# nuclearbombmods/nbody-cosmological-simulation

Measured on AMD Instinct MI355X. Metric: particle-steps/sec (N=65536 fp64 direct-sum leapfrog), higher is better.
Workload: dtype f64

## Files before the change

### nbody_cosmological_simulation_amd/csrc/nb_force_sym.hip

```cpp
#include "nb_dispatch.h"
#include "nb_force_sym_kernel.h"

namespace {


template <typename T, int D, int KICK>
__global__ void __launch_bounds__(NB_BLOCK)
pack_kernel(T *__restrict__ pos, T *__restrict__ vel, const T *__restrict__ acc, const T *__restrict__ mass,
            T *__restrict__ packed, int n, int np, T half_dt, T dt, T gfac, T pad, int p_begin, int p_end, int spread,
            T far_lim, int far_pe)
{
    const int p = p_begin + blockIdx.x * NB_BLOCK + threadIdx.x;
    if (p >= p_end) return;
    if (p < n) {
#pragma unroll
        for (int k = 0; k < D; ++k) {
            const size_t idx = (size_t)p * D + k;
            T x = pos[idx];
            if (KICK) {
                T v = vel[idx];
                if (KICK == NB_PACK_CLOSE_OPEN) v = axpy_rn<T>(v, acc[idx], half_dt);
                v = axpy_rn<T>(v, acc[idx], half_dt);
                x = axpy_rn<T>(x, v, dt);
                vel[idx] = v;
                pos[idx] = x;
            }
            packed[(size_t)k * np + p] = far_pe ? stage_far_pe<T>(x, far_lim, p) : stage_far<T>(x, far_lim, p);
        }
        packed[(size_t)D * np + p] = gfac * mass[p];
    } else {
#pragma unroll
        for (int k = 0; k < D; ++k) packed[(size_t)k * np + p] = (spread && k == 0) ? pad * (T)(1 + (p - n)) : pad;
        packed[(size_t)D * np + p] = (T)0;
    }
}

#ifndef NB_RED_WAVES_N
#define NB_RED_WAVES_N 16
#endif
constexpr int NB_RED_WAVES = NB_RED_WAVES_N;
template <typename T, int D>
__global__ void __launch_bounds__(64 * NB_RED_WAVES)
reduce_sym_kernel(const double *__restrict__ rowslab, const T *__restrict__ colslab,
                  const int *__restrict__ row_slot0, const int *__restrict__ row_nslots,
                  const int *__restrict__ col_upto, int tile_b, int n, int np,
                  double scale, T *__restrict__ acc, T *__restrict__ vel, T half_dt, int do_kick,
                  T *__restrict__ pos, T *__restrict__ packed, T dt, int blk0, double *__restrict__ sums64,
                  double *__restrict__ mm_part, T *__restrict__ pos_next, T far_lim)
{
    __shared__ double s_part[NB_RED_WAVES][D][64];
    const int lane = threadIdx.x & 63, g = threadIdx.x >> 6;
    const int blk = blk0 + blockIdx.x;
    const int p = blk * 64 + lane;
    const int pc = p < n ? p : n - 1;
    const int J = (blk * 64) / tile_b;
    const int s0 = row_slot0[J], ns = row_nslots[J], total = ns + col_upto[J];
    const int off = blk * 64 + lane - J * tile_b;
    double s[D];
#pragma unroll
    for (int k = 0; k < D; ++k) s[k] = 0.0;
#ifndef NB_RED_UNROLL
#define NB_RED_UNROLL 4
#endif
#pragma unroll NB_RED_UNROLL
    for (int c = g; c < total; c += NB_RED_WAVES) {
        if (c < ns) {
#pragma unroll
            for (int k = 0; k < D; ++k) s[k] += rowslab[((size_t)(s0 + c) * D + k) * tile_b + off];
        } else {
#pragma unroll
            for (int k = 0; k < D; ++k) s[k] += (double)colslab[((size_t)(c - ns) * D + k) * np + pc];
        }
    }
#pragma unroll
    for (int k = 0; k < D; ++k) s_part[g][k][lane] = s[k];
    __syncthreads();
    double mm_lo = __builtin_inf(), mm_hi = -__builtin_inf();
    if (g == 0 && p < n) {
#pragma unroll
        for (int k = 0; k < D; ++k) {
            double t = s_part[0][k][lane];
#pragma unroll
            for (int w = 1; w < NB_RED_WAVES; ++w) t += s_part[w][k][lane];
            const size_t idx = (size_t)p * D + k;
            if (sums64) {
                sums64[idx] = t;
                continue;
            }
            const T a = (T)(t * scale);
            const T a_prev = (do_kick & NB_KICK_OPEN_ON_READ) ? acc[idx] : (T)0;
            acc[idx] = a;
            if (mm_part) {
                const double ad = (double)a;
                mm_lo = (ad != ad || mm_lo != mm_lo) ? __builtin_nan("") : (ad < mm_lo ? ad : mm_lo);
                mm_hi = (ad != ad || mm_hi != mm_hi) ? __builtin_nan("") : (ad > mm_hi ? ad : mm_hi);
            }
            const int kmode = do_kick & NB_KICK_MODE_MASK;
            if (kmode != NB_KICK_NONE) {
                T v = vel[idx];
                if (do_kick & NB_KICK_OPEN_ON_READ) v = axpy_rn<T>(v, a_prev, half_dt);
                v = axpy_rn<T>(v, a, half_dt);
                if (kmode == NB_KICK_CLOSE) {
                    vel[idx] = v;
                } else if (kmode == NB_KICK_CLOSE_OPEN) {
                    v = axpy_rn<T>(v, a, half_dt);
                    const T x = axpy_rn<T>(pos[idx], v, dt);
                    vel[idx] = v;
                    pos[idx] = x;
                    packed[(size_t)k * np + p] = stage_far<T>(x, far_lim, p);
                } else {
                    vel[idx] = v;
                    const T vo = axpy_rn<T>(v, a, half_dt);
                    const T x = axpy_rn<T>(pos[idx], vo, dt);
                    pos_next[idx] = x;
                    packed[(size_t)k * np + p] = stage_far<T>(x, far_lim, p);
                }
            }
        }
    }
    if (mm_part && g == 0) {
#pragma unroll
        for (int off = 32; off >= 1; off >>= 1) {
            const double ol = __shfl_xor(mm_lo, off, 64), oh = __shfl_xor(mm_hi, off, 64);
            mm_lo = (ol != ol || mm_lo != mm_lo) ? __builtin_nan("") : (ol < mm_lo ? ol : mm_lo);
            mm_hi = (oh != oh || mm_hi != mm_hi) ? __builtin_nan("") : (oh > mm_hi ? oh : mm_hi);
        }
        if (lane == 0) { mm_part[2 * blockIdx.x] = mm_lo; mm_part[2 * blockIdx.x + 1] = mm_hi; }
    }
}

__global__ void __launch_bounds__(NB_BLOCK)
finish_sums64_kernel(const double *__restrict__ sums64, double scale, float *__restrict__ acc, long long count)
{
    const long long e = (long long)blockIdx.x * NB_BLOCK + threadIdx.x;
    if (e < count) acc[e] = (float)(sums64[e] * scale);
}

template <typename T, typename TM, int D, int R, bool DIAG, bool UNIFORM>
__device__ __forceinline__ double pe_sweep_f64(const T (&xi)[R][D], const TM (&mi)[R], T (&xj)[R][D], TM (&mj)[R], double eps2,
                                               int mass_dt, int rot_addr, int s_begin, int s_count)
{
    double tsum[R];
#pragma unroll
    for (int r = 0; r < R; ++r) tsum[r] = 0.0;
    double half = 0.5, one = 1.0;
    asm volatile("" : "+v"(half), "+s"(one));
#pragma unroll 1
    for (int s = s_begin; s < s_begin + s_count; ++s) {
#pragma unroll
        for (int rj = 0; rj < R; ++rj) {
#pragma unroll
            for (int ri = 0; ri < R; ++ri) {
                double d[D];
#pragma unroll
                for (int k = 0; k < D; ++k) d[k] = (double)xj[rj][k] - (double)xi[ri][k];
                double q = __builtin_fma(d[D - 1], d[D - 1], eps2);
#pragma unroll
                for (int k = D - 2; k >= 0; --k) q = __builtin_fma(d[k], d[k], q);
                const double y0 = __builtin_amdgcn_rsq(q);
                const double e = __builtin_fma(-(q * y0), y0, one);
                const double c = __builtin_fma(e, half, one);
                if (UNIFORM) {
                    if (DIAG && ri == rj) tsum[rj] = (s == 0) ? tsum[rj] : __builtin_fma(y0, c, tsum[rj]);
                    else tsum[rj] = __builtin_fma(y0, c, tsum[rj]);
                } else {
                    double mp;
                    if constexpr (std::is_same_v<TM, float>) mp = (double)mass_prod_f32(mi[ri], mj[rj], mass_dt);
                    else mp = (double)mi[ri] * (double)mj[rj];
                    const double term = mp * (y0 * c);
                    if (DIAG && ri == rj) tsum[rj] += (s == 0) ? 0.0 : term;
                    else tsum[rj] += term;
                }
            }
#pragma unroll
            for (int k = 0; k < D; ++k) xj[rj][k] = rot1<T>(xj[rj][k], rot_addr);
            if (!UNIFORM) mj[rj] = rot1<TM>(mj[rj], rot_addr);
        }
    }
    double tile = tsum[0];
#pragma unroll
    for (int r = 1; r < R; ++r) tile += tsum[r];
    return DIAG ? 0.5 * tile : tile;
}

template <int D, int R, bool DIAG, bool UNIFORM>
__device__ __forceinline__ double pe_sweep_f32(const float (&xi)[R][D], const float (&mi)[R], f2 (&xj2)[R / 2][D], f2 (&mj2)[R / 2],
                                               float eps2, int mass_dt, int rot_addr, int s_begin, int s_count)
{
    f2 ts2[R / 2];
#pragma unroll
    for (int h = 0; h < R / 2; ++h) ts2[h] = f2{0.0f, 0.0f};
#pragma unroll 1
    for (int s = s_begin; s < s_begin + s_count; ++s) {
#pragma unroll
        for (int h = 0; h < R / 2; ++h) {
#pragma unroll
            for (int ri = 0; ri < R; ++ri) {
                f2 d[D];
#pragma unroll
                for (int k = 0; k < D; ++k) d[k] = xj2[h][k] - xi[ri][k];
                f2 r2 = __builtin_elementwise_fma(d[D - 1], d[D - 1], f2{eps2, eps2});
#pragma unroll
                for (int k = D - 2; k >= 0; --k) r2 = __builtin_elementwise_fma(d[k], d[k], r2);
                f2 y = {__builtin_amdgcn_rsqf(r2.x), __builtin_amdgcn_rsqf(r2.y)};
                if (DIAG && s == 0) {
                    if (2 * h == ri) y.x = 0.0f;
                    if (2 * h + 1 == ri) y.y = 0.0f;
                }
                if (UNIFORM) {
                    ts2[h] = ts2[h] + y;
                } else {
                    f2 mp = mj2[h] * mi[ri];
                    if (mass_dt == NB_F16) mp = f2{round_f16(mp.x), round_f16(mp.y)};
// ... 102 lines not shown
                hipLaunchKernelGGL((pack_kernel<T, D.value, K.value>), dim3(grid), dim3(NB_BLOCK), 0, st, (T *)pos, (T *)vel,
                                   (const T *)acc, (const T *)mass, (T *)packed, n, np, (T)half_dt, (T)dt, (T)gfac, (T)pad, p_begin,
                                   p_end, spread_pad, (T)far_lim, far == NB_FAR_PE ? 1 : 0);
                return hipGetLastError();
            });
        });
    });
}

hipError_t nb_launch_force_sym_f64(const double *packed, const SymWork *work, int nwork, double *rowslab,
                                   double *colslab, int np, int dim, int r, int uniform, int pa_f32, double eps2,
                                   hipStream_t st, NbKernelEvents ev, int rowsplit, int ldsrot)
{
    if (ldsrot && dim == 2 && r == 4 && !pa_f32)
        return nb::pick_bool(rowsplit, [&](auto RS) {
            if (ldsrot == SYM_ROT_DPP)
                return launch_sym_ldsrot<RS.value, SYM_ROT_DPP>(packed, work, nwork, rowslab, colslab, np, uniform, eps2, st, ev);
            return launch_sym_ldsrot<RS.value, SYM_ROT_LDS>(packed, work, nwork, rowslab, colslab, np, uniform, eps2, st, ev);
        });
    if (rowsplit) {
        if (dim != 2 || r != 4) return hipErrorInvalidValue;
        if (pa_f32) return launch_sym_rowsplit<HOOK_F32PAIR>(packed, work, nwork, rowslab, colslab, np, uniform, eps2, (float)eps2, st, ev);
        return launch_sym_rowsplit<HOOK_NONE>(packed, work, nwork, rowslab, colslab, np, uniform, eps2, 1.0f, st, ev);
    }
    return nb::pick<2, 3>(dim, [&](auto D) {
        if (pa_f32)
            return nb::pick<2, 4>(r, [&](auto R) {
                return launch_sym_u<double, D.value, R.value, HOOK_F32PAIR>(packed, work, nwork, rowslab, colslab, np, uniform, eps2,
                                                                            nullptr, (float)eps2, st, ev);
            });
        return nb::pick<1, 2, 4>(r, [&](auto R) {
            return launch_sym_u<double, D.value, R.value, HOOK_NONE>(packed, work, nwork, rowslab, colslab, np, uniform, eps2, nullptr,
                                                                     1.0f, st, ev);
        });
    });
}

hipError_t nb_launch_force_sym_f32(const float *packed, const SymWork *work, int nwork, double *rowslab,
                                   float *colslab, int np, int dim, int r, int uniform, int hook, float eps2,
                                   const GridTables *tab, float G, float mass_value, int levels, hipStream_t st,
                                   NbKernelEvents ev)
{
    return nb::pick<2, 3>(dim, [&](auto D) {
        return nb::pick<2, 4>(r, [&](auto R) {
            return nb::pick<HOOK_NONE, HOOK_BF16, HOOK_F16, HOOK_GRID>(hook, [&](auto H) {
                return launch_sym_u<float, D.value, R.value, H.value>(packed, work, nwork, rowslab, colslab, np, uniform, eps2, tab, G,
                                                                      st, ev, mass_value, levels);
            });
        });
    });
}

hipError_t nb_launch_potential_sym(const void *packed, const SymWork *work, int nwork, double *part, int np, int dim,
                                   int r, int is_f64, int f32_terms, int mass_dt, double eps2, int uniform, hipStream_t st)
{
    const float e32 = (float)eps2;
    return nb::pick<2, 3>(dim, [&](auto D) {
        return nb::pick<2, 4>(r, [&](auto R) {
            auto launch = [&](auto real, auto F32T) {
                using T = typename decltype(real)::type;
                return nb::pick_bool(uniform, [&](auto U) {
                    hipLaunchKernelGGL((potential_sym_kernel<T, D.value, R.value, F32T.value, U.value>), dim3(nwork), dim3(NB_BLOCK),
                                       0, st, (const T *)packed, work, part, np, eps2, e32, mass_dt);
                    return hipGetLastError();
                });
            };
            if (is_f64) return nb::pick_bool(f32_terms, [&](auto F32T) { return launch(nb::real_tag<double>{}, F32T); });
            return launch(nb::real_tag<float>{}, std::true_type{});
        });
    });
}

hipError_t nb_launch_finish_sums64(const double *sums64, double scale, float *acc, int64_t count, hipStream_t st)
{
    hipLaunchKernelGGL(finish_sums64_kernel, dim3((unsigned)((count + NB_BLOCK - 1) / NB_BLOCK)), dim3(NB_BLOCK), 0, st, sums64,
                       scale, acc, (long long)count);
    return hipGetLastError();
}

hipError_t nb_launch_reduce_sym(const double *rowslab, const void *colslab, const int *row_slot0,
                                const int *row_nslots, const int *col_upto, int tile_b, int n,
                                int np, int dim, int is_f64, double scale, void *acc, void *vel, double half_dt,
                                int do_kick, void *pos, void *packed, double dt, hipStream_t st, int p_begin, int p_end,
                                double *sums64, double *mm_part, void *pos_next, int far)
{
    const double far_lim = nb_far_limit(far, is_f64);
    if ((do_kick & NB_KICK_MODE_MASK) == NB_KICK_CLOSE_SPEC && !pos_next) return hipErrorInvalidValue;
    if (p_end < 0 || p_end > n) p_end = n;
    if (p_end <= p_begin) return hipSuccess;
    const int blk0 = p_begin / 64;
    const int grid = (p_end + 63) / 64 - blk0;
    return nb::pick<2, 3>(dim, [&](auto D) {
        return nb::pick_real(is_f64, [&](auto real) {
            using T = typename decltype(real)::type;
            hipLaunchKernelGGL((reduce_sym_kernel<T, D.value>), dim3(grid), dim3(64 * NB_RED_WAVES), 0, st, rowslab,
                               (const T *)colslab, row_slot0, row_nslots, col_upto, tile_b, n, np, scale, (T *)acc, (T *)vel,
                               (T)half_dt, do_kick, (T *)pos, (T *)packed, (T)dt, blk0, sums64, mm_part, (T *)pos_next, (T)far_lim);
            return hipGetLastError();
        });
    });
}

#ifdef NB_WG_TRACE
extern "C" int nb_debug_wg_trace(unsigned long long *host, int nwg)
{
    if (nwg > NB_WG_TRACE_MAX) nwg = NB_WG_TRACE_MAX;
    if (hipDeviceSynchronize() != hipSuccess) return -1;
    return hipMemcpyFromSymbol(host, HIP_SYMBOL(nb_wg_trace_buf), sizeof(unsigned long long) * 8 * (size_t)nwg) == hipSuccess ? nwg : -1;
}
#endif
```

### nbody_cosmological_simulation_amd/csrc/nb_internal.h

```cpp
#pragma once
#include <hip/hip_runtime.h>
#include <stdint.h>

#include "../../include/nbody_amd.h"

constexpr int NB_BLOCK = 256;
constexpr int NB_TJ = 256;
constexpr int NB_MAX_LUT = 4096;
constexpr int NB_LUT_MIN = 256;
#ifndef NB_REC_LEVELS
#define NB_REC_LEVELS 32
#endif

enum { HOOK_NONE = 0, HOOK_BF16 = 1, HOOK_F16 = 2, HOOK_GRID = 3,
       HOOK_F32PAIR = 4 ,
       HOOK_AT_RUN_TIME = 5  };

struct GridTables {
    float thr[NB_MAX_LUT + 1];
    float lut[NB_MAX_LUT];
    float qval[NB_MAX_LUT];
    float lmin, lmax, range;
    float r2max;
    float est_a, est_b;
// ... 15 lines not shown
{
    int p = NB_LUT_MIN;
    while (p < levels) p <<= 1;
    return p;
}
inline size_t nb_lut_lds_bytes(int levels) { return 2 * (size_t)(nb_lut_pad(levels) + 1) * sizeof(float); }

struct PruneState {
    unsigned int box_min[3];
    unsigned int box_max[3];
    unsigned long long far;
    unsigned long long lb[2];
    int count;
    int nan_flag;
    int seeded;
    float c[3];
    float rho_m;
    float rho_prev;
    int pair_i, pair_j;
    unsigned int rho_cur;
    unsigned int scan_done;
    unsigned long long best_i, best_j;
};

struct ForceGeom {
    int n;
    int j_begin;
    int j_end;
    int chunk_len;
    int nchunks;
    int r;
};

struct SymWork {
    int tile_i;
    int jt_begin, jt_end;
    int slot;
    int slot_stride;
    int col_ord;
    int s_begin;
    int s_count;
};

enum NbKick {
    NB_KICK_NONE = 0,
    NB_KICK_CLOSE = 1,
    NB_KICK_CLOSE_OPEN = 2,
    NB_KICK_CLOSE_SPEC = 3
};
constexpr int NB_KICK_MODE_MASK = 3;
constexpr int NB_KICK_OPEN_ON_READ = 4;
enum NbPackKick { NB_PACK_NONE = 0, NB_PACK_OPEN = 1, NB_PACK_CLOSE_OPEN = 2 };

struct NbKernelEvents {
    hipEvent_t start = nullptr, stop = nullptr;
};

enum NbFar { NB_FAR_OFF = 0, NB_FAR_FORCE = 1, NB_FAR_PE = 2 };
constexpr double NB_FAR_F64 = 1.2e153;
constexpr float NB_FAR_F32 = 1.2e18f;
inline double nb_far_limit(int far, bool f64_pairs)
{
    if (far == NB_FAR_OFF) return __builtin_inf();
    if (far == NB_FAR_PE && !f64_pairs) return __builtin_inf();
    return f64_pairs ? NB_FAR_F64 : (double)NB_FAR_F32;
}

hipError_t nb_launch_pack(void *pos, void *vel, const void *acc, const void *mass, void *packed, int n, int np,
                          int dim, int is_f64, int kick , double half_dt, double dt, double gfac, int f32_pairs,
                          hipStream_t st, int p_begin = 0, int p_end = -1 ,
                          int spread_pad = 0 ,
                          int far = NB_FAR_FORCE );
hipError_t nb_launch_force_sym_f64(const double *packed, const SymWork *work, int nwork, double *rowslab,
                                   double *colslab, int np, int dim, int r, int uniform, int pa_f32, double eps2,
                                   hipStream_t st, NbKernelEvents ev = {}, int rowsplit = 0 ,
                                   int ldsrot = 0 );
hipError_t nb_launch_force_sym_f32(const float *packed, const SymWork *work, int nwork, double *rowslab,
                                   float *colslab, int np, int dim, int r, int uniform, int hook, float eps2,
                                   const GridTables *tab, float G, float mass_value, int levels, hipStream_t st,
                                   NbKernelEvents ev = {});
hipError_t nb_launch_potential_sym(const void *packed, const SymWork *work, int nwork, double *part, int np, int dim,
                                   int r, int is_f64, int f32_terms, int mass_dt , double eps2,
                                   int uniform , hipStream_t st);
hipError_t nb_launch_final_sum(const double *part, int count, double *out, hipStream_t st);
hipError_t nb_launch_reduce_sym(const double *rowslab, const void *colslab, const int *row_slot0,
                                const int *row_nslots, const int *col_upto, int tile_b, int n,
                                int np, int dim, int is_f64, double scale, void *acc, void *vel, double half_dt,
                                int do_kick ,
                                void *pos, void *packed, double dt, hipStream_t st,
                                int p_begin = 0, int p_end = -1 ,
                                double *sums64 = nullptr ,
                                double *mm_part = nullptr ,
                                void *pos_next = nullptr , int far = NB_FAR_FORCE );
hipError_t nb_launch_finish_sums64(const double *sums64, double scale, float *acc, int64_t count, hipStream_t st);

hipError_t nb_launch_force_f64(const double *pos, const double *mass, double *partial, const ForceGeom &g,
                               int dim, int pair_dt, int qhook, double G, double eps2_py, float eps2_pair,
                               hipStream_t st);
hipError_t nb_launch_force_f32(const float *pos, const float *mass, double *partial, const ForceGeom &g,
                               int dim, int hook, int pa, float G, float eps2, const GridTables *tab, int levels,
                               hipStream_t st, unsigned long long *bin_out = nullptr );
hipError_t nb_launch_force_sym_f32_bins(const float *packed, const SymWork *work, int nwork, double *rowslab,
                                        float *colslab, int np, int dim, int r, int uniform, float eps2,
                                        const GridTables *tab, float G, float mass_value, int levels,
                                        unsigned long long *bin_out, int bin_n, hipStream_t st);
hipError_t nb_launch_grid_quantize_safe_tab(const float *in, float *out, int64_t count, int levels, float min_val,
                                            const double *bounds, GridTables *tab, hipStream_t st);
hipError_t nb_launch_r2max_tables(const float *pos, const ForceGeom &g, int dim, float eps2, GridTables *tab, int levels,
                                  float G, float min_val, int allow_fast, hipStream_t st);
hipError_t nb_launch_r2max(const float *pos, const ForceGeom &g, int dim, float eps2, GridTables *tab,
                           hipStream_t st);
hipError_t nb_launch_r2max_pruned(const float *pos, int n, int dim, float eps2, float *cand, float *rho,
                                  PruneState *ps, GridTables *tab, hipStream_t st);
hipError_t nb_launch_r2max_tracked(const float *pos, int n, int dim, float eps2, float *cand, int *cand_idx, PruneState *ps,
                                   GridTables *tab, int levels, float G, float min_val, int allow_fast, hipStream_t st);
hipError_t nb_launch_grid_tables(GridTables *tab, int levels, float G, float eps2, float min_val,
                                 PruneState *ps , hipStream_t st, int allow_fast = 1);
hipError_t nb_launch_d2bins(const float *pos, int n, int dim, float eps2, const GridTables *tab,
                            int16_t *bins, hipStream_t st, int i0 = 0, int i1 = -1 );

hipError_t nb_launch_reduce(const double *partial, int nchunks, int64_t count, void *acc, int is_f64,
                            void *vel, double half_dt, int do_kick ,
                            void *pos, double dt, hipStream_t st);
hipError_t nb_launch_axpy(void *y, const void *x, double scalar, int64_t count, int is_f64, hipStream_t st);
hipError_t nb_launch_kick_drift(void *pos, void *vel, const void *acc, double half_dt, double dt,
                                int64_t count, int is_f64, hipStream_t st);
hipError_t nb_launch_kick_a32(void *pos, void *vel, const void *acc, double half_dt, double dt, int64_t count,
                              int vel_f64, int pos_f64, int drift, hipStream_t st);
hipError_t nb_launch_convert(const void *in, int in_dt, void *out, int out_dt, int64_t count, hipStream_t st);

hipError_t nb_launch_force_quant_step(float *acc, int64_t count, int levels, double *mn_mx, double *partials,
                                      int16_t *bins, float *vel, float *pos, double half_dt, double dt,
                                      int kick ,
                                      float *packed ,
                                      int np, int dim, hipStream_t st);
hipError_t nb_launch_force_quant_bins(const float *in, float *out, int64_t count, int levels, const double *mn_mx,
                                      int16_t *bins, hipStream_t st);

hipError_t nb_launch_kinetic(const void *vel, const void *mass, int n, int dim, int is_f64, int vel_f32_logical,
                             int half_pa, int mass_dt , double *scratch, double *out,
                             hipStream_t st);
hipError_t nb_launch_potential(const void *pos, const void *mass, const ForceGeom &g, int dim, int is_f64,
                               int pa_f32, int mass_dt , int half_pa, double eps2_py, float eps2_half,
                               double *scratch, double *out, hipStream_t st);

hipError_t nb_launch_cast_hook(const void *in, int in_dt, void *out, int mode, int64_t count, hipStream_t st);
constexpr int NB_MINMAX_BLOCKS = 2048;
hipError_t nb_launch_minmax_generic(const void *in, int is_f64, int64_t count, int log_clamped, double min_val,
                                    double *mn_mx , double *partials, hipStream_t st);
hipError_t nb_launch_grid_quantize(const void *in, void *out, int is_f64, int64_t count, int levels,
                                   const double *mn_mx, hipStream_t st);
hipError_t nb_launch_grid_quantize_safe(const void *in, void *out, int is_f64, int64_t count, int levels,
                                        double min_val, const double *mn_mx, hipStream_t st);

struct NbMetricsArgs {
    const void *pos, *vel, *mass;
    int n, dim;
    int storage_f64;
    int arith_f64;
    int num_bins;
    const float *edges;
    double max_radius;
    int kth;
    double G;
    int radius_only;
    void *scratch;
    double *out;
};
size_t nb_metrics_scratch_bytes(int n, int num_bins);
size_t nb_sort_temp_bytes(int n, int key64);
hipError_t nb_sort_keys(void *tmp, size_t tmp_bytes, const void *kin, void *kout, int n, int key64, hipStream_t st);
hipError_t nb_sort_pairs(void *tmp, size_t tmp_bytes, const void *kin, void *kout, const int *vin, int *vout, int n,
                         int key64, hipStream_t st);
hipError_t nb_launch_metrics(const NbMetricsArgs &a, hipStream_t st);

size_t nb_p2p_handle_bytes();
// ... 102 lines not shown
```

### nbody_cosmological_simulation_amd/csrc/nb_plan.cpp

```cpp
#include "nb_plan.h"

#include <algorithm>
#include <cmath>
#include <cstdlib>

namespace {
int env_int(const char *name, int dflt)
{
    const char *e = getenv(name);
    return e ? atoi(e) : dflt;
}
}

NbKnobs nb_read_knobs()
{
    NbKnobs k;
    k.sym = env_int("NB_SYM", -1);
    k.sym_r = env_int("NB_SYM_R", 0);
    k.sym_cl = std::max(0, env_int("NB_SYM_CL", 0));
    k.sym_split = env_int("NB_SYM_SPLIT", 0);
    if (k.sym_split < 1 || k.sym_split > 16) k.sym_split = 0;
    k.sym_rowsplit = env_int("NB_SYM_ROWSPLIT", -1);
    if (k.sym_rowsplit > 8) k.sym_rowsplit = -1;
    k.tail_pieces = env_int("NB_SYM_TAIL", 0);
    if (k.tail_pieces != 2 && k.tail_pieces != 4 && k.tail_pieces != 8 && k.tail_pieces != 16) k.tail_pieces = 0;
    k.sym_rot = env_int("NB_SYM_ROT", -1);
    if (k.sym_rot < 0 || k.sym_rot > 2) k.sym_rot = -1;
    k.r_onesided = env_int("NB_R", 0);
    k.no_prune = getenv("NB_NO_PRUNE") != nullptr;
    k.no_track = env_int("NB_NO_TRACK", 0) != 0;
    k.no_pe_sym = getenv("NB_NO_PE_SYM") != nullptr;
    k.no_uniform = getenv("NB_NO_UNIFORM") != nullptr;
    k.no_smalln = getenv("NB_NO_SMALLN") != nullptr;
    k.no_grid_fast = getenv("NB_NO_GRID_FAST") != nullptr;
    k.no_p2p = getenv("NB_NO_P2P") != nullptr;
    k.no_p2p_kick = getenv("NB_P2P_NO_KICK") != nullptr;
    k.no_small_fuse = getenv("NB_NO_SMALL_FUSE") != nullptr;
    k.no_spec = getenv("NB_NO_SPEC") != nullptr;
    k.no_x64 = getenv("NB_NO_X64") != nullptr;
    k.no_red_mm = getenv("NB_NO_RED_MM") != nullptr;
    k.small_max = std::max(0, env_int("NB_SMALL_MAX", 0));
    k.small_lanes = env_int("NB_SMALL_LANES", 0);
    if (k.small_lanes != 16 && k.small_lanes != 32 && k.small_lanes != 64) k.small_lanes = 0;
    return k;
}

void nb_plan_sym(const PlanInput &in, const NbKnobs &knobs, SymPlanHost &sp)
{
    sp = SymPlanHost();
    const int n = in.n, dim = in.dim, P = in.nranks;
    const bool is_f64 = in.is_f64;
    const bool tiny = is_f64 && dim == 2 && n <= 2816;
    const int sym_from = dim == 3 ? (is_f64 ? 8192 : 4096) : (is_f64 ? 5120 : 1024);
    int want = (tiny || n >= sym_from) ? 1 : 0;
    if (knobs.sym >= 0) want = knobs.sym;
    if (!want || ((in.flags & NB_FLAG_NO_COMM) && want < 2)) return;
    if (is_f64 && in.mode != NB_FLOAT64) return;
    sp.r = tiny ? 1 : (n >= 20480 || is_f64) ? 4 : 2;
    if ((knobs.sym_r == 1 && is_f64 && dim == 2) || knobs.sym_r == 2 || knobs.sym_r == 4) sp.r = knobs.sym_r;
    sp.tile_b = 64 * sp.r;
    const int T = (n + sp.tile_b - 1) / sp.tile_b;
    const int SR = (T + 3) / 4;
    sp.tiles = SR * 4;
    sp.np = sp.tiles * sp.tile_b;
    const size_t el = is_f64 ? sizeof(double) : sizeof(float);
    if (SR < P) return;
    {
        const long long rows_max = (SR + P - 1) / P;
        const long long entries_max = knobs.sym_split ? rows_max * knobs.sym_split
                                                      : rows_max + 7 * std::min<long long>(rows_max, 2LL * in.cus);
        if ((size_t)dim * sp.np * el * (size_t)entries_max > (size_t)48 << 30) return;
    }

    std::vector<int> ord(SR, -1);
    sp.row_slot0.assign(sp.tiles, 0);
    sp.row_nslots.assign(sp.tiles, 0);
    long long owned_pairs = 0;
    int nrows = 0;
    for (int S = 0; S < SR; ++S) {
        const int k = S % (2 * P);
        const int owner = k < P ? k : 2 * P - 1 - k;
        if (owner == in.rank) {
            ord[S] = nrows++;
            for (int w = 0; w < 4; ++w) owned_pairs += std::max(0, T - (4 * S + w));
        }
    }
    const long long target_items = is_f64 ? 2048 : 4096;
    int cl = (int)(owned_pairs / target_items / 4);
    cl = std::max(1, std::min(cl, 16));
    if (knobs.sym_cl > 0) cl = knobs.sym_cl;
    sp.cl = cl;

    const long long wg_slots = 4LL * in.cus;
    std::vector<int> nch_of(SR, 0), split_of(SR, 1);
    long long items = 0;
    for (int S = 0; S < SR; ++S)
        if (ord[S] >= 0) { nch_of[S] = (T - 4 * S + cl - 1) / cl; items += nch_of[S]; }
    int rowsplit = 0;
    if (knobs.sym_split) {
        for (int S = 0; S < SR; ++S) split_of[S] = knobs.sym_split;
    } else if (sp.r == 4 && items < 1000) {
        int pieces = 4;
        {
            const double t_step[4] = {0.70, 0.60, 0.62, 0.55};
            double best = 1e30;
            for (int nsp : {2, 3, 4, 5, 6, 8}) {
                if (items >= 500 && nsp != 4) continue;
                const long long wgs = items * nsp, rounds = (wgs + in.cus - 1) / in.cus;
                const double cost = rounds * ((64 + nsp - 1) / nsp + 1) * t_step[std::min<long long>(rounds, 4) - 1] +
                                    0.3 * 5.0 * (double)wgs / in.cus;
                if (cost < best) { best = cost; pieces = nsp; }
            }
            if (is_f64 && dim == 2 && cl == 1 && knobs.sym_rowsplit != 0) {
                long long rows_units = 0;
                for (int S = 0; S < SR; ++S)
                    if (ord[S] >= 0) for (int w = 0; w < 4; ++w) rows_units += std::max(0, T - (4 * S + w));
                for (int nsp : {1, 2, 3, 4}) {
                    const long long wgs = rows_units * nsp, rounds = (wgs + in.cus - 1) / in.cus;
                    const double cost = rounds * ((64 + 4 * nsp - 1) / (4 * nsp) + 1) * t_step[std::min<long long>(rounds, 4) - 1] +
                                        0.5 * 2.0 * (double)wgs / in.cus;
                    if (cost < best) { best = cost; rowsplit = nsp; }
                }
            }
// ... 77 lines not shown
```

### nbody_cosmological_simulation_amd/csrc/nb_plan.h

```cpp
#pragma once
#include <vector>

#include "nb_internal.h"

#ifndef NB_SYM_ROT_DEFAULT
#define NB_SYM_ROT_DEFAULT 2
#endif

struct NbKnobs {
    int sym = -1;
    int sym_r = 0;
    int sym_cl = 0;
    int sym_split = 0;
    int sym_rowsplit = -1;
    int tail_pieces = 0;
    int sym_rot = -1;
    int r_onesided = 0;
    bool no_prune = false;
    bool no_track = false;
    bool no_pe_sym = false;
    bool no_uniform = false;
    bool no_smalln = false;
    int small_max = 0;
    int small_lanes = 0;
    bool no_grid_fast = false;
    bool no_p2p = false;
    bool no_red_mm = false;
    bool no_x64 = false;
    bool no_small_fuse = false;
    bool no_p2p_kick = false;
    bool no_spec = false;
};
NbKnobs nb_read_knobs();

struct SymPlanHost {
    bool enabled = false;
    int r = 2, tile_b = 128, tiles = 0, np = 0, nslots = 0, ncol = 0, cl = 1;
    int rowsplit = 0;
    std::vector<SymWork> work;
    std::vector<int> row_slot0, row_nslots, col_upto;
    size_t col_bytes = 0, row_bytes = 0, packed_bytes = 0;
};

struct PlanInput {
    int n = 0, dim = 2, mode = 0, flags = 0, rank = 0, nranks = 1;
    bool is_f64 = true;
    bool multi = false;
    int cus = 256;
};

void nb_plan_sym(const PlanInput &in, const NbKnobs &knobs, SymPlanHost &out);
```

### nbody_cosmological_simulation_amd/csrc/nb_step.cpp

```cpp
#include <algorithm>
#include <cstring>

#include "nb_state.h"

namespace nbhost {

struct NbTuning {
    int onesided_r1_max_n = 8192;
    int onesided_target_wgs = 1024;
    int prune_min_n = 8192;
    int track_min_n = 3072;
    int red_mm_max_blocks = 1024;
    int small_max_f64 = 4096;
    int small_max_f32 = 3072;
    int small_fuse_tables_max_n = 2048;
};
static const NbTuning g_tune{};

int small_max_n(bool is_f64) { return is_f64 ? g_tune.small_max_f64 : g_tune.small_max_f32; }

int onesided_r(int n, const NbKnobs &knobs)
{
    if (knobs.r_onesided == 1 || knobs.r_onesided == 2 || knobs.r_onesided == 4)
        return knobs.r_onesided;
// ... 250 lines not shown
            if (int rc = comm_allreduce_max_u32(s, &s->tab->r2max_bits)) return rc;
    }
    HIPCHK(nb_launch_grid_tables(s->tab, L, G, e.eps2, min_val, prune ? s->prune_state : nullptr, s->stream, allow_fast(s)));
    s->prune_seeded = prune;
    return NB_OK;
}

int launch_pairs(nb_sim *s, const EvalRequest &rq, const Eval &e)
{
    const nb_config &c = s->cfg;
    const auto &sp = s->sym;
    const bool grid = e.hook == HOOK_GRID;
    const int L = grid ? mode_levels(c) : 0;
    unsigned long long *bin_out = (rq.bins && grid) ? s->bin_out : nullptr;
    int slot;
    if (!e.used_sym) {
        if (int rc = prof_begin(s, &slot)) return rc;
        if (s->is_f64)
            HIPCHK(nb_launch_force_f64((const double *)s->pos, (const double *)s->mass, s->partial, s->geom, c.dim, e.pair_dt,
                                       e.hook, c.G, c.softening_sq, e.eps2, s->stream));
        else
            HIPCHK(nb_launch_force_f32((const float *)s->pos, (const float *)s->mass, s->partial, s->geom, c.dim, e.hook,
                                       e.pair_dt, (float)c.G, e.eps2, s->tab, L, s->stream, bin_out));
        s->last_kernel = s->is_f64 ? "force_f64_kernel" : "force_f32_kernel";
        return prof_end(s, slot);
    }
    const int pa_f32 = s->is_f64 && e.pair_dt == NB_F32;
    if (!rq.packed_ready) {
        const double gfac = s->is_f64 ? c.G : (grid ? 1.0 : (double)(float)c.G);
        HIPCHK(nb_launch_pack(s->pos, s->vel, s->acc, s->mass, sp.packed, c.n, sp.np, c.dim, s->is_f64, NB_PACK_NONE, 0.0, 0.0,
                              gfac, pa_f32, s->stream, 0, -1, 0, grid ? NB_FAR_OFF : NB_FAR_FORCE));
    }
    if (int rc = prof_begin(s, &slot, false)) return rc;
    if (s->is_f64) {
        HIPCHK(nb_launch_force_sym_f64((const double *)sp.packed, sp.work, sp.nwork, sp.rowslab, (double *)sp.colslab, sp.np,
                                       c.dim, sp.r, s->mass_uniform, pa_f32, c.softening_sq, s->stream, prof_events(s, slot),
                                       sp.rowsplit ? 1 : 0, s->knobs.sym_rot >= 0 ? s->knobs.sym_rot : NB_SYM_ROT_DEFAULT));
        s->last_kernel = "force_sym_kernel<double";
        return NB_OK;
    }
    const bool uniform = grid ? (s->mass_uniform && sp.r != 2) : e.sym_uniform;
    if (bin_out)
        HIPCHK(nb_launch_force_sym_f32_bins((const float *)sp.packed, sp.work, sp.nwork, sp.rowslab, (float *)sp.colslab, sp.np,
                                            c.dim, sp.r, uniform, e.eps2, s->tab, (float)c.G, (float)s->mass_value, L, bin_out,
                                            c.n, s->stream));
    else
        HIPCHK(nb_launch_force_sym_f32((const float *)sp.packed, sp.work, sp.nwork, sp.rowslab, (float *)sp.colslab, sp.np,
                                       c.dim, sp.r, uniform, e.hook, e.eps2, s->tab, (float)c.G, (float)s->mass_value, L,
                                       s->stream, prof_events(s, slot)));
    s->last_kernel = "force_sym_kernel<float";
    return NB_OK;
}

int reduce_and_exchange(nb_sim *s, const EvalRequest &rq, Eval &e, EvalResult *res)
{
    const nb_config &c = s->cfg;
    const int64_t cnt = nd(s);
    const bool p2p = e.multi && (e.x64 ? p2p_use_x64(s, cnt) : p2p_use(s, cnt));
    void *red_out = p2p ? nb_p2p_data() : (rq.bins ? s->staging : s->acc);
    if (e.x64 && !p2p && !s->sums64) HIPCHK(hipMalloc((void **)&s->sums64, (size_t)cnt * sizeof(double)));
    double *sums64 = e.x64 ? (p2p ? (double *)nb_p2p_data() : s->sums64) : nullptr;
    if (p2p)
        if (int rc = p2p_claim_buffer(s)) return rc;
    const bool fuse_kick = rq.kick && !e.multi && !e.fq;
    int kmode = kick_mode(fuse_kick, rq.open_next);
    if (rq.open_on_read && !(fuse_kick && e.used_sym))
        return fail(NB_ERR_INVALID, "internal: a step started from speculative positions needs the kick-fusing pair-symmetric reduction");
    if (!e.used_sym) {
        HIPCHK(nb_launch_reduce(s->partial, s->geom.nchunks, cnt, red_out, s->is_f64, s->vel, c.dt / 2, kmode, s->pos, c.dt,
                                s->stream));
        site_set(res, "reduce", kmode);
    } else {
        const auto &sp = s->sym;
        if (e.sym_uniform) e.scale = s->is_f64 ? c.G * s->mass_value : (double)((float)c.G * (float)s->mass_value);
        const bool spec = kmode == NB_KICK_CLOSE && rq.spec_next && !grid_mode(c.mode);
        if (spec) {
            if (!s->pos_alt) HIPCHK(hipMalloc(&s->pos_alt, (size_t)cnt * (s->is_f64 ? 8 : 4)));
            kmode = NB_KICK_CLOSE_SPEC;
        }
        if (rq.open_on_read) kmode |= NB_KICK_OPEN_ON_READ;
        HIPCHK(nb_launch_reduce_sym(sp.rowslab, sp.colslab, sp.row_slot0, sp.row_nslots, sp.col_upto, sp.tile_b, c.n, sp.np,
                                    c.dim, s->is_f64, e.scale, red_out, s->vel, c.dt / 2, kmode, s->pos, sp.packed, c.dt,
                                    s->stream, 0, -1, sums64, e.red_mm ? s->scalars + 8 : nullptr, s->pos_alt,
                                    grid_mode(c.mode) ? NB_FAR_OFF : NB_FAR_FORCE));
        site_set(res, "reduce_sym", kmode);
        if (spec) { s->spec_open = true; s->spec_kind = 2; s->spec_dt = c.dt; }
    }
    e.kicked = fuse_kick;
    res->opened = (kmode & NB_KICK_MODE_MASK) == NB_KICK_CLOSE_OPEN;
    if (p2p) {
        NbP2PKick kk{};
        kk.scale = e.scale;
        if (e.x64) kk.f64_to_f32 = 1;
        else if (rq.kick && !e.fq && !s->knobs.no_p2p_kick) {
            kk.mode = kick_mode(true, rq.open_next);
            kk.dim = c.dim; kk.np = e.used_sym ? s->sym.np : 0;
            kk.vel = s->vel; kk.pos = s->pos; kk.packed = e.used_sym ? (void *)s->sym.packed : nullptr;
            kk.half_dt = c.dt / 2; kk.dt = c.dt;
            kk.far_lim = nb_far_limit(grid_mode(c.mode) ? NB_FAR_OFF : NB_FAR_FORCE, s->is_f64);
            e.kicked = true;
            res->opened = rq.open_next;
        }
        HIPCHK(nb_p2p_allreduce(s->acc, (size_t)cnt, s->is_f64 || e.x64, p2p_step_timeout_s(), s->stream, &kk));
        if (kk.mode != NB_KICK_NONE) site_set(res, "p2p", kk.mode);
        s->used_p2p = true;
    } else if (e.x64) {
        if (int rc = comm_allreduce_sum(s, s->sums64, (size_t)cnt, true)) return rc;
        HIPCHK(nb_launch_finish_sums64(s->sums64, e.scale, (float *)s->acc, cnt, s->stream));
    } else if (e.multi) {
        if (int rc = comm_allreduce_sum(s, s->acc, (size_t)cnt, s->is_f64)) return rc;
    }
    return NB_OK;
}

int force_quant_finish(nb_sim *s, const EvalRequest &rq, Eval &e, EvalResult *res)
{
    const nb_config &c = s->cfg;
    const int km = kick_mode(rq.kick, rq.open_next);
    if (e.red_mm)
        HIPCHK(nb_launch_force_quant_finish((float *)s->acc, nd(s), mode_levels(c), s->scalars + 8, (c.n + 63) / 64, s->scalars,
                                            s->fbins, (float *)s->vel, (float *)s->pos, c.dt / 2, c.dt, km, s->stream,
                                            (float *)s->sym.packed, s->sym.np, c.dim));
    else
        HIPCHK(nb_launch_force_quant_step((float *)s->acc, nd(s), mode_levels(c), s->scalars, s->scalars + 8, s->fbins,
                                          (float *)s->vel, (float *)s->pos, c.dt / 2, c.dt, km,
                                          e.used_sym ? (float *)s->sym.packed : nullptr, s->sym.np, c.dim, s->stream));
    const bool packed = km == NB_KICK_CLOSE_OPEN && e.used_sym;
    site_set(res, "fq_finish", km, packed ? (e.red_mm ? ",packed,red_mm" : ",packed") : (e.red_mm ? ",red_mm" : ""));
    e.kicked = rq.kick;
    res->opened = rq.open_next;
    return NB_OK;
}

}

int force_eval(nb_sim *s, EvalRequest rq, EvalResult *result)
{
    if (!s->have_pos || !s->have_mass) return fail(NB_ERR_INVALID, "positions and masses must be set first");
    rq.open_next = rq.kick && rq.open_next;
    EvalResult unread;
    EvalResult *res = result ? result : &unread;
    *res = EvalResult{};
    Eval e = resolve_eval(s);
    if (e.multi && !s->comm) return fail(NB_ERR_COMM, "nranks > 1 but nb_comm_init was not called");
    if (e.multi)
        if (int rc = comm_check(s)) return rc;
    if (e.shard && rq.kick) return fail(NB_ERR_INVALID, "NB_FLAG_NO_COMM handles cannot step");
    if (e.generic) return force_eval_generic(s, rq, e, res);
    s->last_generic = false;
    if (rq.bins) e.fq = e.red_mm = false;
    if (e.hook == HOOK_GRID)
        if (int rc = grid_prepare(s, e, false)) return rc;
    if (int rc = launch_pairs(s, rq, e)) return rc;
    if (int rc = reduce_and_exchange(s, rq, e, res)) return rc;
    if (e.fq)
        if (int rc = force_quant_finish(s, rq, e, res)) return rc;
    if (rq.kick && !e.kicked) {
        if (rq.may_defer) res->deferred = true;
        else {
            HIPCHK(nb_launch_axpy(s->vel, s->acc, s->cfg.dt / 2, nd(s), s->is_f64, s->stream));
            snprintf(res->site, sizeof res->site, "axpy");
        }
    }
    if (rq.bins) return NB_OK;
    s->logical[3] = acc_logical_dtype(s);
    s->have_acc = true;
    return NB_OK;
// ... 271 lines not shown
```

Baseline: 57.65 million.

## Add multi-chain reduce_sym kernel with per-wave independent accumulators and unrolled loads

Adds a new reduce_sym_chains kernel in which each wave keeps CH independent partial-sum chains and issues U batches of slab loads before adding. This exposes more memory-level parallelism and shortens dependent add chains in the row/column slab reduction. It is selected by default (4 waves, 4 chains, 2 unrolls for fp64), with the classic kernel still available through an env knob. Fewer waves per block and more registers per thread may reduce occupancy. The reduction is a small part of the step next to the O(N^2) force pass.

```diff
diff --git a/nbody_cosmological_simulation_amd/csrc/nb_force_sym.hip b/nbody_cosmological_simulation_amd/csrc/nb_force_sym.hip
--- a/nbody_cosmological_simulation_amd/csrc/nb_force_sym.hip
+++ b/nbody_cosmological_simulation_amd/csrc/nb_force_sym.hip
@@ -39,6 +39,7 @@
 #define NB_RED_WAVES_N 16
 #endif
 constexpr int NB_RED_WAVES = NB_RED_WAVES_N;
+constexpr int NB_RED_SHAPE_F64 = 402, NB_RED_SHAPE_F32 = 401;
 template <typename T, int D>
 __global__ void __launch_bounds__(64 * NB_RED_WAVES)
 reduce_sym_kernel(const double *__restrict__ rowslab, const T *__restrict__ colslab,
@@ -129,6 +130,225 @@
     }
 }
 
+template <typename T, int D>
+struct RedSlot {
+    double r[D];
+    T c[D];
+};
+template <int D>
+struct RedSlot<double, D> {
+    double r[D];
+};
+
+template <int KIND, typename T, int D>
+__device__ __forceinline__ void red_load(RedSlot<T, D> &v, int c, const double *__restrict__ rowslab,
+                                         const T *__restrict__ colslab, int s0, int ns, int tile_b, int np, int off, int pc)
+{
+    const bool row = KIND == 1 || (KIND == 0 && c < ns);
+    if (row) {
+#pragma unroll
+        for (int k = 0; k < D; ++k) v.r[k] = rowslab[((size_t)(s0 + c) * D + k) * tile_b + off];
+    } else if constexpr (std::is_same_v<T, double>) {
+#pragma unroll
+        for (int k = 0; k < D; ++k) v.r[k] = colslab[((size_t)(c - ns) * D + k) * np + pc];
+    } else {
+#pragma unroll
+        for (int k = 0; k < D; ++k) v.c[k] = colslab[((size_t)(c - ns) * D + k) * np + pc];
+    }
+}
+
+template <int KIND, typename T, int D>
+__device__ __forceinline__ void red_add(double (&s)[D], const RedSlot<T, D> &v, int c, int ns)
+{
+    if constexpr (std::is_same_v<T, double>) {
+#pragma unroll
+        for (int k = 0; k < D; ++k) s[k] += v.r[k];
+    } else {
+        const bool row = KIND == 1 || (KIND == 0 && c < ns);
+        if (row) {
+#pragma unroll
+            for (int k = 0; k < D; ++k) s[k] += v.r[k];
+        } else {
+#pragma unroll
+            for (int k = 0; k < D; ++k) s[k] += (double)v.c[k];
+        }
+    }
+}
+
+template <int KIND, typename T, int D, int CH, int U>
+__device__ __forceinline__ void red_trip(double (&s)[CH][D], int base, const double *__restrict__ rowslab,
+                                         const T *__restrict__ colslab, int s0, int ns, int tile_b, int np, int off, int pc)
+{
+    RedSlot<T, D> v[U][CH];
+#pragma unroll
+    for (int u = 0; u < U; ++u)
+#pragma unroll
+        for (int j = 0; j < CH; ++j) red_load<KIND, T, D>(v[u][j], base + 16 * u + j, rowslab, colslab, s0, ns, tile_b, np, off, pc);
+#pragma unroll
+    for (int u = 0; u < U; ++u)
+#pragma unroll
+        for (int j = 0; j < CH; ++j) red_add<KIND, T, D>(s[j], v[u][j], base + 16 * u + j, ns);
+}
+
+template <typename T>
+__device__ __forceinline__ T red_finish(double t, double scale, int do_kick, size_t idx, int k, int p, int np, T v0, T x0,
+                                        T a_prev, T half_dt, T dt, T far_lim, T *__restrict__ acc, T *__restrict__ vel,
+                                        T *__restrict__ pos, T *__restrict__ packed, T *__restrict__ pos_next)
+{
+    const T a = (T)(t * scale);
+    acc[idx] = a;
+    const int kmode = do_kick & NB_KICK_MODE_MASK;
+    if (kmode != NB_KICK_NONE) {
+        T v = v0;
+        if (do_kick & NB_KICK_OPEN_ON_READ) v = axpy_rn<T>(v, a_prev, half_dt);
+        v = axpy_rn<T>(v, a, half_dt);
+        if (kmode == NB_KICK_CLOSE) {
+            vel[idx] = v;
+        } else if (kmode == NB_KICK_CLOSE_OPEN) {
+            v = axpy_rn<T>(v, a, half_dt);
+            const T x = axpy_rn<T>(x0, v, dt);
+            vel[idx] = v;
+            pos[idx] = x;
+            packed[(size_t)k * np + p] = stage_far<T>(x, far_lim, p);
+        } else {
+            vel[idx] = v;
+            const T vo = axpy_rn<T>(v, a, half_dt);
+            const T x = axpy_rn<T>(x0, vo, dt);
+            pos_next[idx] = x;
+            packed[(size_t)k * np + p] = stage_far<T>(x, far_lim, p);
+        }
+    }
+    return a;
+}
+
+__device__ __forceinline__ void red_mm_take(double &mm_lo, double &mm_hi, double ad)
+{
+    mm_lo = (ad != ad || mm_lo != mm_lo) ? __builtin_nan("") : (ad < mm_lo ? ad : mm_lo);
+    mm_hi = (ad != ad || mm_hi != mm_hi) ? __builtin_nan("") : (ad > mm_hi ? ad : mm_hi);
+}
+
+template <typename T, int D, int CH, int U>
+__global__ void __launch_bounds__(64 * (16 / CH))
+reduce_sym_chains_kernel(const double *__restrict__ rowslab, const T *__restrict__ colslab,
+                         const int *__restrict__ row_slot0, const int *__restrict__ row_nslots,
+                         const int *__restrict__ col_upto, int tile_b, int n, int np,
+                         double scale, T *__restrict__ acc, T *__restrict__ vel, T half_dt, int do_kick,
+                         T *__restrict__ pos, T *__restrict__ packed, T dt, int blk0, double *__restrict__ sums64,
+                         double *__restrict__ mm_part, T *__restrict__ pos_next, T far_lim)
+{
+    constexpr int NW = 16 / CH;
+    constexpr int FD = NW == 1 ? D : 1;
+    static_assert(NW == 1 || NW >= D, "wave k finishes component k");
+    __shared__ double s_part[NW == 1 ? 1 : 16][D][64];
+    __shared__ double s_acc[NW == 1 ? 1 : D][64];
+    const int lane = threadIdx.x & 63, w = threadIdx.x >> 6, g0 = w * CH;
+    const int blk = blk0 + blockIdx.x;
+    const int p = blk * 64 + lane;
+    const int pc = p < n ? p : n - 1;
+    const int J = (blk * 64) / tile_b;
+    const int s0 = row_slot0[J], ns = row_nslots[J], total = ns + col_upto[J];
+    const int off = blk * 64 + lane - J * tile_b;
+
+    const bool fin = p < n && (NW == 1 || w < D);
+    const int kmode = do_kick & NB_KICK_MODE_MASK;
+    T v0[FD], x0[FD], a_prev[FD];
+#pragma unroll
+    for (int f = 0; f < FD; ++f) {
+        const size_t idx = (size_t)pc * D + (NW == 1 ? f : (w < D ? w : 0));
+        v0[f] = (fin && !sums64 && kmode != NB_KICK_NONE) ? vel[idx] : (T)0;
+        x0[f] = (fin && !sums64 && (kmode == NB_KICK_CLOSE_OPEN || kmode == NB_KICK_CLOSE_SPEC)) ? pos[idx] : (T)0;
+        a_prev[f] = (fin && !sums64 && (do_kick & NB_KICK_OPEN_ON_READ)) ? acc[idx] : (T)0;
+    }
+
+    double s[CH][D];
+#pragma unroll
+    for (int j = 0; j < CH; ++j)
+#pragma unroll
+        for (int k = 0; k < D; ++k) s[j][k] = 0.0;
+    for (int base = g0; base < total; base += 16 * U) {
+        const int last = base + 16 * (U - 1) + CH - 1;
+        if (last < ns) {
+            red_trip<1, T, D, CH, U>(s, base, rowslab, colslab, s0, ns, tile_b, np, off, pc);
+        } else if (base >= ns && last < total) {
+            red_trip<2, T, D, CH, U>(s, base, rowslab, colslab, s0, ns, tile_b, np, off, pc);
+        } else {
+            RedSlot<T, D> v[U][CH];
+#pragma unroll
+            for (int u = 0; u < U; ++u)
+#pragma unroll
+                for (int j = 0; j < CH; ++j) {
+                    const int c = base + 16 * u + j;
+                    if (c < total) red_load<0, T, D>(v[u][j], c, rowslab, colslab, s0, ns, tile_b, np, off, pc);
+                }
+#pragma unroll
+            for (int u = 0; u < U; ++u)
+#pragma unroll
+                for (int j = 0; j < CH; ++j) {
+                    const int c = base + 16 * u + j;
+                    if (c < total) red_add<0, T, D>(s[j], v[u][j], c, ns);
+                }
+        }
+    }
+
+    double t[FD];
+    if constexpr (NW == 1) {
+#pragma unroll
+        for (int k = 0; k < D; ++k) {
+            t[k] = s[0][k];
+#pragma unroll
+            for (int j = 1; j < 16; ++j) t[k] += s[j][k];
+        }
+    } else {
+#pragma unroll
+        for (int j = 0; j < CH; ++j)
+#pragma unroll
+            for (int k = 0; k < D; ++k) s_part[g0 + j][k][lane] = s[j][k];
+        __syncthreads();
+        if (w < D) {
+            t[0] = s_part[0][w][lane];
+#pragma unroll
+            for (int g = 1; g < 16; ++g) t[0] += s_part[g][w][lane];
+        }
+    }
+
+    double mm_lo = __builtin_inf(), mm_hi = -__builtin_inf();
+    if (fin) {
+#pragma unroll
+        for (int f = 0; f < FD; ++f) {
+            const int k = NW == 1 ? f : w;
+            const size_t idx = (size_t)p * D + k;
+            if (sums64) {
+                sums64[idx] = t[f];
+                continue;
+            }
+            const T a = red_finish<T>(t[f], scale, do_kick, idx, k, p, np, v0[f], x0[f], a_prev[f], half_dt, dt, far_lim, acc,
+                                      vel, pos, packed, pos_next);
+            if (mm_part) {
+                if (NW == 1 || w == 0) red_mm_take(mm_lo, mm_hi, (double)a);
+                else s_acc[w][lane] = (double)a;
+            }
+        }
+    }
+    if (mm_part) {
+        if constexpr (NW > 1) {
+            __syncthreads();
+            if (w == 0 && p < n && !sums64) {
+#pragma unroll
+                for (int k = 1; k < D; ++k) red_mm_take(mm_lo, mm_hi, s_acc[k][lane]);
+            }
+        }
+        if (w == 0) {
+#pragma unroll
+            for (int o = 32; o >= 1; o >>= 1) {
+                const double ol = __shfl_xor(mm_lo, o, 64), oh = __shfl_xor(mm_hi, o, 64);
+                mm_lo = (ol != ol || mm_lo != mm_lo) ? __builtin_nan("") : (ol < mm_lo ? ol : mm_lo);
+                mm_hi = (oh != oh || mm_hi != mm_hi) ? __builtin_nan("") : (oh > mm_hi ? oh : mm_hi);
+            }
+            if (lane == 0) { mm_part[2 * blockIdx.x] = mm_lo; mm_part[2 * blockIdx.x + 1] = mm_hi; }
+        }
+    }
+}
+
 __global__ void __launch_bounds__(NB_BLOCK)
 finish_sums64_kernel(const double *__restrict__ sums64, double scale, float *__restrict__ acc, long long count)
 {
@@ -397,7 +617,7 @@
                                 const int *row_nslots, const int *col_upto, int tile_b, int n,
                                 int np, int dim, int is_f64, double scale, void *acc, void *vel, double half_dt,
                                 int do_kick, void *pos, void *packed, double dt, hipStream_t st, int p_begin, int p_end,
-                                double *sums64, double *mm_part, void *pos_next, int far)
+                                double *sums64, double *mm_part, void *pos_next, int far, int shape)
 {
     const double far_lim = nb_far_limit(far, is_f64);
     if ((do_kick & NB_KICK_MODE_MASK) == NB_KICK_CLOSE_SPEC && !pos_next) return hipErrorInvalidValue;
@@ -405,13 +625,25 @@
     if (p_end <= p_begin) return hipSuccess;
     const int blk0 = p_begin / 64;
     const int grid = (p_end + 63) / 64 - blk0;
+    if (shape == NB_RED_AUTO) shape = is_f64 ? NB_RED_SHAPE_F64 : NB_RED_SHAPE_F32;
     return nb::pick<2, 3>(dim, [&](auto D) {
         return nb::pick_real(is_f64, [&](auto real) {
             using T = typename decltype(real)::type;
-            hipLaunchKernelGGL((reduce_sym_kernel<T, D.value>), dim3(grid), dim3(64 * NB_RED_WAVES), 0, st, rowslab,
-                               (const T *)colslab, row_slot0, row_nslots, col_upto, tile_b, n, np, scale, (T *)acc, (T *)vel,
-                               (T)half_dt, do_kick, (T *)pos, (T *)packed, (T)dt, blk0, sums64, mm_part, (T *)pos_next, (T)far_lim);
-            return hipGetLastError();
+            if (shape == NB_RED_CLASSIC) {
+                hipLaunchKernelGGL((reduce_sym_kernel<T, D.value>), dim3(grid), dim3(64 * NB_RED_WAVES), 0, st, rowslab,
+                                   (const T *)colslab, row_slot0, row_nslots, col_upto, tile_b, n, np, scale, (T *)acc, (T *)vel,
+                                   (T)half_dt, do_kick, (T *)pos, (T *)packed, (T)dt, blk0, sums64, mm_part, (T *)pos_next,
+                                   (T)far_lim);
+                return hipGetLastError();
+            }
+            return nb::pick<104, 401, 402, 1601>(shape, [&](auto S) {
+                constexpr int CH = S.value / 100, U = S.value % 100;
+                hipLaunchKernelGGL((reduce_sym_chains_kernel<T, D.value, CH, U>), dim3(grid), dim3(64 * (16 / CH)), 0, st,
+                                   rowslab, (const T *)colslab, row_slot0, row_nslots, col_upto, tile_b, n, np, scale, (T *)acc,
+                                   (T *)vel, (T)half_dt, do_kick, (T *)pos, (T *)packed, (T)dt, blk0, sums64, mm_part,
+                                   (T *)pos_next, (T)far_lim);
+                return hipGetLastError();
+            });
         });
     });
 }
diff --git a/nbody_cosmological_simulation_amd/csrc/nb_internal.h b/nbody_cosmological_simulation_amd/csrc/nb_internal.h
--- a/nbody_cosmological_simulation_amd/csrc/nb_internal.h
+++ b/nbody_cosmological_simulation_amd/csrc/nb_internal.h
@@ -121,6 +121,7 @@
 hipError_t nb_launch_potential_sym(const void *packed, const SymWork *work, int nwork, double *part, int np, int dim,
                                    int r, int is_f64, int f32_terms, int mass_dt , double eps2,
                                    int uniform , hipStream_t st);
+constexpr int NB_RED_AUTO = 0, NB_RED_CLASSIC = -1;
 hipError_t nb_launch_final_sum(const double *part, int count, double *out, hipStream_t st);
 hipError_t nb_launch_reduce_sym(const double *rowslab, const void *colslab, const int *row_slot0,
                                 const int *row_nslots, const int *col_upto, int tile_b, int n,
@@ -130,7 +131,8 @@
                                 int p_begin = 0, int p_end = -1 ,
                                 double *sums64 = nullptr ,
                                 double *mm_part = nullptr ,
-                                void *pos_next = nullptr , int far = NB_FAR_FORCE );
+                                void *pos_next = nullptr , int far = NB_FAR_FORCE ,
+                                int shape = NB_RED_AUTO );
 hipError_t nb_launch_finish_sums64(const double *sums64, double scale, float *acc, int64_t count, hipStream_t st);
 
 hipError_t nb_launch_force_f64(const double *pos, const double *mass, double *partial, const ForceGeom &g,
diff --git a/nbody_cosmological_simulation_amd/csrc/nb_plan.cpp b/nbody_cosmological_simulation_amd/csrc/nb_plan.cpp
--- a/nbody_cosmological_simulation_amd/csrc/nb_plan.cpp
+++ b/nbody_cosmological_simulation_amd/csrc/nb_plan.cpp
@@ -39,6 +39,9 @@
     k.no_spec = getenv("NB_NO_SPEC") != nullptr;
     k.no_x64 = getenv("NB_NO_X64") != nullptr;
     k.no_red_mm = getenv("NB_NO_RED_MM") != nullptr;
+    k.red_shape = env_int("NB_RED_SHAPE", 0);
+    if (k.red_shape != 104 && k.red_shape != 401 && k.red_shape != 402 && k.red_shape != 1601) k.red_shape = NB_RED_AUTO;
+    if (env_int("NB_RED_CLASSIC", 0) != 0) k.red_shape = NB_RED_CLASSIC;
     k.small_max = std::max(0, env_int("NB_SMALL_MAX", 0));
     k.small_lanes = env_int("NB_SMALL_LANES", 0);
     if (k.small_lanes != 16 && k.small_lanes != 32 && k.small_lanes != 64) k.small_lanes = 0;
diff --git a/nbody_cosmological_simulation_amd/csrc/nb_plan.h b/nbody_cosmological_simulation_amd/csrc/nb_plan.h
--- a/nbody_cosmological_simulation_amd/csrc/nb_plan.h
+++ b/nbody_cosmological_simulation_amd/csrc/nb_plan.h
@@ -30,6 +30,7 @@
     bool no_small_fuse = false;
     bool no_p2p_kick = false;
     bool no_spec = false;
+    int red_shape = 0;
 };
 NbKnobs nb_read_knobs();
 
diff --git a/nbody_cosmological_simulation_amd/csrc/nb_step.cpp b/nbody_cosmological_simulation_amd/csrc/nb_step.cpp
--- a/nbody_cosmological_simulation_amd/csrc/nb_step.cpp
+++ b/nbody_cosmological_simulation_amd/csrc/nb_step.cpp
@@ -356,7 +356,7 @@
         HIPCHK(nb_launch_reduce_sym(sp.rowslab, sp.colslab, sp.row_slot0, sp.row_nslots, sp.col_upto, sp.tile_b, c.n, sp.np,
                                     c.dim, s->is_f64, e.scale, red_out, s->vel, c.dt / 2, kmode, s->pos, sp.packed, c.dt,
                                     s->stream, 0, -1, sums64, e.red_mm ? s->scalars + 8 : nullptr, s->pos_alt,
-                                    grid_mode(c.mode) ? NB_FAR_OFF : NB_FAR_FORCE));
+                                    grid_mode(c.mode) ? NB_FAR_OFF : NB_FAR_FORCE, s->knobs.red_shape));
         site_set(res, "reduce_sym", kmode);
         if (spec) { s->spec_open = true; s->spec_kind = 2; s->spec_dt = c.dt; }
     }
```

Measured after the change: 57.80 million, median of 6. No clear change (+0.2%).
